# Chemical118/TREW

Hardware: NVIDIA B200
Metric: Gbases/s for trew short 5 32 at 1/2/4/8 B200; % of HBM roofline (higher is better)
Workload: dtype u64

## Files before the change

### trew_b200/csrc/device_ctx.cu

```cuda
#include <algorithm>
#include <chrono>
#include <cstdarg>
#include <cstdio>
#include <cstdlib>
#include <cstring>
#include <string>
#include <thread>
#include <vector>

#include <cuda_runtime.h>

#include "host_internal.h"
#include "scan_kernels.cuh"

using namespace trew;

namespace {

template <typename T, bool Pinned = false>
struct Buf {
    T* p = nullptr;
    size_t cap = 0;
    Buf() = default;
    Buf(Buf&& o) noexcept : p(o.p), cap(o.cap) { o.p = nullptr; o.cap = 0; }
    Buf(const Buf&) = delete;
    Buf& operator=(const Buf&) = delete;
    ~Buf() { release(); }
    cudaError_t grow(size_t n, cudaStream_t st) {
        if (n <= cap) return cudaSuccess;
        if (p) { cudaError_t e = cudaStreamSynchronize(st); if (e != cudaSuccess) return e; }
        return alloc(std::max((n + n / 4) * sizeof(T), (size_t)1 << 20) / sizeof(T));
    }
    cudaError_t alloc(size_t n) {
        cudaError_t e = release();
        if (e == cudaSuccess) e = Pinned ? cudaHostAlloc((void**)&p, n * sizeof(T), cudaHostAllocDefault) : cudaMalloc((void**)&p, n * sizeof(T));
        if (e != cudaSuccess) p = nullptr;
        else cap = n;
        return e;
    }
    cudaError_t release() {
        cudaError_t e = cudaSuccess;
        if (p) e = Pinned ? cudaFreeHost(p) : cudaFree(p);
        p = nullptr; cap = 0;
        return e;
    }
};

constexpr int kScanCounters = 8;
struct ScanBufs {
    Buf<unsigned int> survivors, counters;
    Buf<unsigned char> scratch;
    cudaError_t alloc(uint32_t n_units) {
        cudaError_t e = survivors.alloc(2 * (size_t)std::max<uint32_t>(n_units, 1));
        return e == cudaSuccess ? counters.alloc(kScanCounters) : e;
    }
};

struct SlotRes {
    Buf<unsigned char, true> h_buf;
    Buf<unsigned char> d_buf;
    Buf<unsigned char, true> h_inv;
    Buf<unsigned char> d_inv;
    size_t inv_cap = 0;
    Buf<unsigned int, true> h_keys;
    ScanBufs scan;
    size_t survivors_cap = 0;
    cudaStream_t stream = nullptr;
    cudaEvent_t ev_start = nullptr, ev_done = nullptr;
    bool in_flight = false;
};

struct RangeInfo { uint32_t r0, r1; uint64_t bases; uint32_t max_len; };

}

struct trew_resident {
    Buf<unsigned char> d_buf;
    DevBatch batch{};
    uint32_t n_reads = 0, n_units = 0, max_read_len = 0;
    uint64_t bases = 0;
    ScanBufs scan;
    cudaEvent_t ev[4] = {nullptr, nullptr, nullptr, nullptr};
    bool ev_pending = false;
};

struct trew_ctx {
    trew_config cfg{};
    int sm_count = 0;
    LaunchPlan plan{};
    cudaStream_t aux_stream = nullptr;
    cudaEvent_t ev_join = nullptr;
    int resident_streams = 1;
    uint64_t resident_seq = 0;
    DevCfg dcfg{};
    size_t n_slots = 0;
    Buf<Slot> table;
// ... 457 lines not shown
    return check_batch(nullptr, mode, batch);
}

static thread_local std::string g_create_error;

static int default_host_threads(int asked) {
    return asked > 0 ? asked : (int)std::min(64u, std::max(1u, std::thread::hardware_concurrency()));
}

const char* trew_dev_last_error(const trew_ctx* ctx) { return ctx ? ctx->err.c_str() : g_create_error.c_str(); }

static int create_ctx(const trew_config* cfg, trew_ctx** out, std::string& g_create_error, Pool* shared_pool) {
    if (!cfg || !out) return TREW_ERR_ARG;
    *out = nullptr;
    g_create_error.clear();
    auto bad_arg = [&](const char* msg) { g_create_error = msg; return TREW_ERR_ARG; };
    if (cfg->mode < 0 || cfg->mode > 2) return bad_arg("mode must be TREW_MODE_SHORT, _PAIR or _LONG");
    if (cfg->min_mer < 3 || cfg->max_mer > 64 || cfg->min_mer > cfg->max_mer) return bad_arg("need 3 <= MIN_MER <= MAX_MER <= 64");
    if (!(0 < cfg->low_baseline && cfg->low_baseline <= 1) || !(0 < cfg->high_baseline && cfg->high_baseline <= 1) ||
        cfg->low_baseline > cfg->high_baseline) return bad_arg("need 0 < LOW_BASELINE <= HIGH_BASELINE <= 1");
    if (cfg->mode == TREW_MODE_LONG && cfg->slice_length > 0 && cfg->slice_length < 2 * cfg->max_mer)
        return bad_arg("SLICE_LENGTH must be greater than or equal to twice of MAX_MER.");
    if (cfg->mode == TREW_MODE_LONG && cfg->slice_length > 512)
        return bad_arg("SLICE_LENGTH above 512 is not supported by the GPU path (a slice of up to 2*SLICE_LENGTH-1 bases must fit "
                       "a 1023-base window); use -s 512 or less.");
    trew_ctx* ctx = new trew_ctx();
    ctx->cfg = *cfg;
    if (ctx->cfg.slice_length <= 0) ctx->cfg.slice_length = 150;
    auto bail = [&](int rc) { g_create_error = ctx->err; trew_dev_destroy(ctx); return rc; };
#define CKC(call)                                                                                   \
    do {                                                                                            \
        cudaError_t e_ = (call);                                                                    \
        if (e_ != cudaSuccess) { fail(ctx, TREW_ERR_CUDA, "%s: %s", #call, cudaGetErrorString(e_)); return bail(TREW_ERR_CUDA); } \
    } while (0)
    const bool timing = getenv("TREW_CLI_TIMING") != nullptr;
    auto now = [] { return std::chrono::duration<double, std::milli>(std::chrono::steady_clock::now().time_since_epoch()).count(); };
    double t_prev = now();
    auto lap = [&](const char* what) {
        if (!timing) return;
        const double t = now();
        fprintf(stderr, "[trew] create, device %d: %s %.1f ms\n", cfg->device, what, t - t_prev);
        t_prev = t;
    };
    int ndev = 0;
    CKC(cudaGetDeviceCount(&ndev));
    lap("driver init");
    if (cfg->device < 0 || cfg->device >= ndev) { fail(ctx, TREW_ERR_CUDA, "no CUDA device %d (found %d)", cfg->device, ndev); return bail(TREW_ERR_CUDA); }
    CKC(cudaSetDevice(cfg->device));
    cudaDeviceProp prop;
    CKC(cudaGetDeviceProperties(&prop, cfg->device));
    ctx->sm_count = prop.multiProcessorCount;
    ctx->plan = default_launch_plan(ctx->sm_count);
    {
        auto env_int = [](const char* name, int dflt) { const char* e = getenv(name); return e && *e ? atoi(e) : dflt; };
        int v;
        if ((v = env_int("TREW_GRID_SCREEN", 0)) > 0) ctx->plan.screen_blocks = ctx->sm_count * v;
        if ((v = env_int("TREW_GRID_DECIDE", 0)) > 0) ctx->plan.decide_blocks = ctx->sm_count * v;
        if ((v = env_int("TREW_GRID_EXACT", 0)) > 0) ctx->plan.exact_blocks = std::min(ctx->plan.exact_blocks, ctx->sm_count * v);
        ctx->resident_streams = env_int("TREW_RESIDENT_STREAMS", 1) >= 2 ? 2 : 1;
        ctx->sparse_val = env_int("TREW_DENSE_VAL", 0) == 0;
        ctx->exact_flags = (unsigned int)env_int("TREW_EXACT_FLAGS", 0);
    }
    int lg = cfg->table_log2_slots > 0 ? cfg->table_log2_slots : 22;
    if (lg < 10 || lg > 28) { fail(ctx, TREW_ERR_ARG, "table_log2_slots out of range"); return bail(TREW_ERR_ARG); }
    ctx->n_slots = (size_t)1 << lg;
    CKC(ctx->table.alloc(ctx->n_slots));
    CKC(cudaMemset(ctx->table.p, 0, ctx->n_slots * sizeof(Slot)));
    lap("primary context + count table");
    CKC(ctx->d_error.alloc(2));
    CKC(cudaMemset(ctx->d_error.p, 0, 2 * sizeof(unsigned int)));
    CKC(ctx->d_total_surv.alloc(1));
    CKC(cudaMemset(ctx->d_total_surv.p, 0, sizeof(unsigned long long)));
    std::vector<unsigned short> thr;
    build_thr(cfg->low_baseline, thr);
    std::vector<unsigned short> thr_hi;
    build_thr(cfg->high_baseline, thr_hi);
    CKC(ctx->d_thr.alloc(2 * thr.size()));
    CKC(cudaMemcpy(ctx->d_thr.p, thr.data(), thr.size() * sizeof(unsigned short), cudaMemcpyHostToDevice));
    CKC(cudaMemcpy(ctx->d_thr.p + thr.size(), thr_hi.data(), thr_hi.size() * sizeof(unsigned short), cudaMemcpyHostToDevice));
    ctx->dcfg.mode = cfg->mode; ctx->dcfg.min_mer = cfg->min_mer; ctx->dcfg.max_mer = cfg->max_mer;
    ctx->dcfg.slice_len = ctx->cfg.slice_length; ctx->dcfg.low = cfg->low_baseline; ctx->dcfg.high = cfg->high_baseline;
    ctx->dcfg.slots = ctx->table.p; ctx->dcfg.slot_mask = (unsigned int)(ctx->n_slots - 1);
    ctx->dcfg.error_flag = ctx->d_error.p; ctx->dcfg.thr_low = ctx->d_thr.p; ctx->dcfg.thr_high = ctx->d_thr.p + kThrTableSize;
    CKC(prepare_exact(kMaxWindow + 9));
    lap("kernel attributes (module load)");
    CKC(cudaStreamCreateWithFlags(&ctx->main_stream, cudaStreamNonBlocking));
    CKC(cudaStreamCreateWithFlags(&ctx->aux_stream, cudaStreamNonBlocking));
    CKC(cudaEventCreateWithFlags(&ctx->ev_join, cudaEventDisableTiming));
    CKC(cudaEventCreate(&ctx->ev_a));
    CKC(cudaEventCreate(&ctx->ev_b));
    CKC(cudaEventCreate(&ctx->ev_t0));
    CKC(cudaEventCreate(&ctx->ev_t1));
    ctx->staging_bytes = cfg->staging_bytes ? (size_t)cfg->staging_bytes : ((size_t)64 << 20);
    int ns = cfg->n_staging > 0 ? cfg->n_staging : 3;
    ctx->slots.resize((size_t)ns);
    for (auto& s : ctx->slots) {
        CKC(s.h_buf.alloc(ctx->staging_bytes));
        CKC(s.d_buf.alloc(ctx->staging_bytes));
        s.inv_cap = ctx->staging_bytes / 8 / kInvRecBytes;
        CKC(s.h_inv.alloc((s.inv_cap + 1) * kInvRecBytes));
        CKC(s.d_inv.alloc((s.inv_cap + 1) * kInvRecBytes));
        CKC(s.h_keys.alloc(1));
        *s.h_keys.p = 0;
        s.survivors_cap = ctx->staging_bytes / 8;
        CKC(s.scan.alloc((uint32_t)s.survivors_cap));
        CKC(cudaStreamCreateWithFlags(&s.stream, cudaStreamNonBlocking));
        CKC(cudaEventCreate(&s.ev_start));
        CKC(cudaEventCreate(&s.ev_done));
    }
    CKC(ctx->d_n.alloc(1));
    lap("staging ring (pinned + device buffers)");
    if (shared_pool) { ctx->pool = shared_pool; ctx->own_pool = false; }
    else ctx->pool = new Pool(default_host_threads(cfg->host_threads));
#undef CKC
    *out = ctx;
    return TREW_OK;
}

int trew_dev_create(const trew_config* cfg, trew_ctx** out) { return create_ctx(cfg, out, g_create_error, nullptr); }

void trew_dev_destroy(trew_ctx* ctx) {
    if (!ctx) return;
    cudaSetDevice(ctx->cfg.device);
    cudaDeviceSynchronize();
    for (auto& s : ctx->slots) {
        if (s.stream) cudaStreamDestroy(s.stream);
        if (s.ev_start) cudaEventDestroy(s.ev_start);
        if (s.ev_done) cudaEventDestroy(s.ev_done);
    }
    if (ctx->main_stream) cudaStreamDestroy(ctx->main_stream);
    if (ctx->aux_stream) cudaStreamDestroy(ctx->aux_stream);
    if (ctx->ev_join) cudaEventDestroy(ctx->ev_join);
    if (ctx->ev_a) cudaEventDestroy(ctx->ev_a);
    if (ctx->ev_b) cudaEventDestroy(ctx->ev_b);
    if (ctx->ev_t0) cudaEventDestroy(ctx->ev_t0);
    if (ctx->ev_t1) cudaEventDestroy(ctx->ev_t1);
    if (ctx->own_pool) delete ctx->pool;
    delete ctx;
}

int trew_dev_submit_chunk(trew_ctx* ctx, const char* buffer1, const int32_t* locs1, uint32_t n1,
                          const char* buffer2, const int32_t* locs2, uint32_t n2) {
    if (!ctx) return TREW_ERR_ARG;
    CK(cudaSetDevice(ctx->cfg.device));
    const bool pair = ctx->cfg.mode == TREW_MODE_PAIR;
    if (pair ? (!buffer2 && n2) : (buffer2 != nullptr || n2 != 0)) return fail(ctx, TREW_ERR_ARG, "second chunk only in pair mode");
    if ((n1 && (!buffer1 || !locs1)) || (n2 && !locs2)) return fail(ctx, TREW_ERR_ARG, "null chunk");
    ChunkView cv{{buffer1, buffer2}, {locs1, locs2}, {nullptr, nullptr}, pair ? 2u : 1u};
    const uint32_t n = pair ? 2u * std::min(n1, n2) : n1;
    if (n == 0) return TREW_OK;
    for (int sd = 0; sd < (pair ? 2 : 1); sd++) {
        const int32_t* l = cv.locs[sd];
        uint32_t cnt = pair ? n / 2 : n;
        int32_t last = l[2 * (size_t)(cnt - 1) + 1];
        if (last >= l[2 * (size_t)(cnt - 1)]) cv.end[sd] = cv.buf[sd] + last + 1;
    }
    return submit_chunk_view(ctx, cv, n);
}

int trew_dev_submit_packed(trew_ctx* ctx, const trew_batch* batch) {
    if (!ctx || !batch) return TREW_ERR_ARG;
    int rc = check_batch(ctx, ctx->cfg.mode, batch);
    if (rc) return rc;
    CK(cudaSetDevice(ctx->cfg.device));
    uint32_t n = batch->n_reads;
    if (n == 0) return TREW_OK;
// ... 629 lines not shown
```

### trew_b200/csrc/scan_kernels.cu

```cuda
#include "scan_kernels.cuh"
#include "exact_thread.cuh"

#include <cstdio>

namespace trew {

typedef unsigned int u32;
typedef unsigned long long u64;
typedef unsigned __int128 u128;


__device__ __forceinline__ u32 lane_id() { return threadIdx.x & 31; }

__device__ __forceinline__ u32 low_mask(int bits) {
    return bits >= 32 ? 0xffffffffu : ((1u << bits) - 1u);
}

__device__ __forceinline__ u32 prefix_xor32(u32 x) {
    x ^= x << 1; x ^= x << 2; x ^= x << 4; x ^= x << 8; x ^= x << 16;
    return x;
}

__device__ __forceinline__ u64 mix64(u64 x) {
    x ^= x >> 33; x *= 0xff51afd7ed558ccdULL; x ^= x >> 33; x *= 0xc4ceb9fe1a85ec53ULL; x ^= x >> 33;
    return x;
}


__device__ __noinline__ void table_add_impl(Slot* slots, u32 slot_mask, u32* error_flag, u32 meta, u64 lo, u64 hi, u64 cnt) {
#ifdef TREW_EXP_NOADD
    return;
#endif
    u64 h = mix64(lo ^ mix64(hi + 0x9e3779b97f4a7c15ULL * (u64)(meta + 1)));
    u32 i = (u32)h & slot_mask;
    for (u32 probe = 0; probe <= slot_mask; probe++, i = (i + 1) & slot_mask) {
        Slot* s = slots + i;
        const uint4 a = __ldcg(reinterpret_cast<const uint4*>(s)), c = __ldcg(reinterpret_cast<const uint4*>(s) + 1);
        u32 st = c.w;
        if (st == 2u) {
            if (c.z == meta && a.x == (u32)lo && a.y == (u32)(lo >> 32) && a.z == (u32)hi && a.w == (u32)(hi >> 32)) {
                atomicAdd(&s->count, cnt);
                return;
            }
            __threadfence();
            if (__ldcg(&s->meta) == meta && __ldcg(&s->seq_lo) == lo && __ldcg(&s->seq_hi) == hi) {
                atomicAdd(&s->count, cnt);
                return;
            }
            continue;
        }
        int outcome = 0;
        do {
            st = atomicCAS(&s->state, 0u, 1u);
            if (st == 0u) {
                s->seq_lo = lo; s->seq_hi = hi; s->meta = meta;
                __threadfence();
                atomicExch(&s->state, 2u);
                atomicAdd(&s->count, cnt);
                atomicAdd(error_flag + 1, 1u);
                outcome = 1;
            } else if (st == 2u) {
                __threadfence();
                if (__ldcg(&s->meta) == meta && __ldcg(&s->seq_lo) == lo && __ldcg(&s->seq_hi) == hi) {
                    atomicAdd(&s->count, cnt);
                    outcome = 1;
                } else outcome = 2;
            }
        } while (outcome == 0);
        if (outcome == 1) return;
    }
    atomicExch(error_flag, 3u);
}

__device__ __forceinline__ void rec_append(UnitRecs* R, u64 unit, int table, int k, u64 lo, u64 hi, u64 count) {
    const u32 act = __activemask(), lane = threadIdx.x & 31;
    const int leader = __ffs(act) - 1;
    u64 base = 0;
    if ((int)lane == leader) base = atomicAdd(&R->n, (u64)__popc(act));
    base = __shfl_sync(act, base, leader);
    const u64 i = base + (u64)__popc(act & ((1u << lane) - 1u));
    if (i < R->cap) {
        uint4* p = reinterpret_cast<uint4*>(R->buf + i);
        p[0] = make_uint4((u32)unit, (u32)(unit >> 32), (u32)lo, (u32)(lo >> 32));
        p[1] = make_uint4((u32)hi, (u32)(hi >> 32), (u32)count, (u32)table | ((u32)k << 8));
// ... 202 lines not shown
        csa(x[0], x[1], x[2], s1, c1); csa(x[3], x[4], x[5], s2, c2); csa(s1, s2, x[6], s3, c3);
        csa(c1, c2, c3, s4, c4);
        return __popc(s3) + __popc(x[7]) + 2 * __popc(s4) + 4 * __popc(c4);
    } else {
        int t = 0;
#pragma unroll
        for (int j = 0; j < NW; j++) t += __popc(x[j]);
        return t;
    }
}

template <int NW>
__device__ __noinline__ bool probe_filter(const DevBatch& b, u32 pos, int wl, int k0, int k1,
                                          const unsigned short* __restrict__ thr) {
    u32 PH[NW], PL[NW], QH[NW], QL[NW], WV[NW];
    {
        u32 t[NW];
        load_bits<NW>(b.hi, pos, t); prefix_xor_excl<NW>(t, PH);
        load_bits<NW>(b.lo, pos, t); prefix_xor_excl<NW>(t, PL);
        load_bits<NW>(b.val, pos, WV); mask_bits<NW>(WV, wl);
    }
    shr_var<NW>(PH, k0, QH);
    shr_var<NW>(PL, k0, QL);
    sliding_and<NW>(WV, k0);
    u32 PA[NW];
    bool have_pa = false;
    for (int k = k0; k <= k1; k++) {
        u32 a[NW], bb[NW], c[NW];
#pragma unroll
        for (int j = 0; j < NW; j++) {
            u32 dh = QH[j] ^ PH[j], dl = QL[j] ^ PL[j];
            a[j] = dh & WV[j]; bb[j] = dl & WV[j]; c[j] = a[j] & dl;
        }
        int T = popc_multi<NW>(WV);
        if (T == 0) break;
        int cH = popc_multi<NW>(a), cL = popc_multi<NW>(bb), c11 = popc_multi<NW>(c);
        int c10 = cH - c11, c01 = cL - c11, c00 = T - cH - cL + c11;
        int U = max(max(c00, c01), max(c10, c11));
        int need = thr[T];
        if (U >= need) {
            u32 QA[NW];
            if (!have_pa) {
                u32 A[NW], t[NW];
                load_bits<NW>(b.hi, pos, A); load_bits<NW>(b.lo, pos, t);
#pragma unroll
                for (int j = 0; j < NW; j++) A[j] &= t[j];
                prefix_xor_excl<NW>(A, PA);
                have_pa = true;
            }
            shr_var<NW>(PA, k, QA);
            u32 x11[NW], x10[NW], x01[NW], x00[NW];
#pragma unroll
            for (int j = 0; j < NW; j++) {
                u32 da = QA[j] ^ PA[j];
                u32 dh = QH[j] ^ PH[j], dl = QL[j] ^ PL[j];
                x11[j] = c[j] & da; x10[j] = a[j] & ~dl & da; x01[j] = bb[j] & ~dh & da; x00[j] = WV[j] & ~dh & ~dl & da;
            }
            int n11 = popc_multi<NW>(x11), n10 = popc_multi<NW>(x10), n01 = popc_multi<NW>(x01), n00 = popc_multi<NW>(x00);
            int U2 = max(max(max(n11, c11 - n11), max(n10, c10 - n10)), max(max(n01, c01 - n01), max(n00, c00 - n00)));
            if (U2 >= need) return true;
        }
        shr1<NW>(QH); shr1<NW>(QL);
        u32 t[NW];
#pragma unroll
        for (int j = 0; j < NW; j++) t[j] = WV[j];
        shr1<NW>(t);
#pragma unroll
        for (int j = 0; j < NW; j++) WV[j] &= t[j];
    }
    return false;
}

template <int MAXNW>
__device__ __forceinline__ bool probe_dispatch(const DevBatch& b, const Probe& p, const unsigned short* thr) {
    if (p.k1 < p.k0) return false;
    int need_bits = p.wl + 1;
    if (need_bits <= 96) return probe_filter<3>(b, p.pos, p.wl, p.k0, p.k1, thr);
    if constexpr (MAXNW >= 5) { if (need_bits <= 160) return probe_filter<5>(b, p.pos, p.wl, p.k0, p.k1, thr); }
    if constexpr (MAXNW >= 8) { if (need_bits <= 256) return probe_filter<8>(b, p.pos, p.wl, p.k0, p.k1, thr); }
    return true;
}


constexpr u32 kPackC11 = 1u - (1u << 8) - (1u << 16) + (1u << 24);
constexpr u32 kPackH = (1u << 8) - (1u << 24);
constexpr u32 kPackL = (1u << 16) - (1u << 24);
#ifndef TREW_SCREEN_UNROLL
#define TREW_SCREEN_UNROLL 2
#endif
constexpr int kScreenUnroll = TREW_SCREEN_UNROLL;
constexpr int kFastMaxWl = 95;
constexpr int kFastTabSize = kFastMaxWl + 2;
constexpr int kProbeShift = 28;
constexpr int kMod4BelowWindows = 48;
constexpr int kThreadMinWindows = 36;

__device__ __forceinline__ uint4 fast_entry(int T, int need) {
    uint4 e = make_uint4(0u, 0u, 0u, 0u);
    if (T <= 0) return e;
    int T01 = min(T, 64);
    e.y = T >= 32 ? 0xffffffffu : ((1u << T) - 1u);
    e.z = T <= 32 ? 0u : (T >= 64 ? 0xffffffffu : ((1u << (T - 32)) - 1u));
    int np = need - (T - T01);
    if (np <= 0) e.x = 0x80808080u;
    else if (np > 64) e.x = (u32)T01 << 24;
    else e.x = ((u32)T01 << 24) + (u32)(128 - np) * 0x01010101u;
    return e;
}

template <int S>
__device__ __forceinline__ bool fast_span(const u32 (&ph)[5], const u32 (&pl)[5], int wl, int ka, int kb,
                                          const uint4* __restrict__ tab) {
    const uint4* tp = tab + (wl - ka + 1);
#pragma unroll (kScreenUnroll)
    for (int k = ka; k <= kb; k++, tp--) {
        const uint4 e = *tp;
        u32 qh0 = __funnelshift_r(ph[S], ph[S + 1], k), qh1 = __funnelshift_r(ph[S + 1], ph[S + 2], k);
        u32 ql0 = __funnelshift_r(pl[S], pl[S + 1], k), ql1 = __funnelshift_r(pl[S + 1], pl[S + 2], k);
        u32 a0 = (qh0 ^ ph[0]) & e.y, a1 = (qh1 ^ ph[1]) & e.z;
        u32 b0 = (ql0 ^ pl[0]) & e.y, b1 = (ql1 ^ pl[1]) & e.z;
        u32 x = e.x + (u32)(__popc(a0) + __popc(a1)) * kPackH + (u32)(__popc(b0) + __popc(b1)) * kPackL +
                (u32)(__popc(a0 & b0) + __popc(a1 & b1)) * kPackC11;
        if (x & 0x80808080u) return true;
    }
    return false;
}

__device__ __forceinline__ bool probe_is_fast(const Probe& p) { return p.wl <= kFastMaxWl && p.k1 <= 63 && p.k1 <= p.wl; }

__device__ __forceinline__ bool screen_probe(const DevBatch& b, const Probe& p, const uint4* __restrict__ tab) {
    if (p.k1 < p.k0) return false;
    if (!probe_is_fast(p)) return true;
    u32 t[3], full[3] = {0xffffffffu, 0xffffffffu, 0xffffffffu};
    mask_bits<3>(full, p.wl);
    load_bits<3>(b.val, p.pos, t);
    if ((((t[0] & full[0]) ^ full[0]) | ((t[1] & full[1]) ^ full[1]) | ((t[2] & full[2]) ^ full[2])) != 0u) return true;
    u32 ph[5], pl[5], q[3];
    load_bits<3>(b.hi, p.pos, t); mask_bits<3>(t, p.wl); prefix_xor_excl<3>(t, q);
    ph[0] = q[0]; ph[1] = q[1]; ph[2] = q[2]; ph[3] = 0u; ph[4] = 0u;
    load_bits<3>(b.lo, p.pos, t); mask_bits<3>(t, p.wl); prefix_xor_excl<3>(t, q);
    pl[0] = q[0]; pl[1] = q[1]; pl[2] = q[2]; pl[3] = 0u; pl[4] = 0u;
    int k0 = p.k0;
    if (k0 < 32) {
        if (fast_span<0>(ph, pl, p.wl, k0, min(p.k1, 31), tab)) return true;
        k0 = 32;
    }
    return p.k1 >= 32 && fast_span<1>(ph, pl, p.wl, k0, p.k1, tab);
}

constexpr int kFastMaxWlLong = 159;
constexpr int kFastTabSizeLong = kFastMaxWlLong + 2;
struct __align__(16) FastEntryLong { u32 base, m0, m1, m2, m3, pad0, pad1, pad2; };

__device__ __forceinline__ FastEntryLong fast_entry_long(int T, int need) {
    FastEntryLong e = {0u, 0u, 0u, 0u, 0u, 0u, 0u, 0u};
    if (T <= 0) return e;
    const int T01 = min(T, 128);
    u32 m[4];
#pragma unroll
    for (int j = 0; j < 4; j++) { int vb = T - 32 * j; m[j] = vb <= 0 ? 0u : low_mask(min(32, vb)); }
    e.m0 = m[0]; e.m1 = m[1]; e.m2 = m[2]; e.m3 = m[3];
    const int np = need - (T - T01);
    if (np <= 0) e.base = 0x80808080u;
    else if (np > 128) e.base = 0u;
    else e.base = ((u32)T01 << 24) + (u32)(128 - np) * 0x01010101u;
    return e;
}

template <int S>
__device__ __forceinline__ bool fast_span_long(const u32 (&ph)[8], const u32 (&pl)[8], int wl, int ka, int kb,
                                               const FastEntryLong* __restrict__ tab) {
    const FastEntryLong* tp = tab + (wl - ka + 1);
    for (int k = ka; k <= kb; k++, tp--) {
        const uint4 e0 = *reinterpret_cast<const uint4*>(tp);
        const u32 m3 = tp->m3;
        if (e0.x == 0u) continue;
        const u32 mk[4] = {e0.y, e0.z, e0.w, m3};
        int cH = 0, cL = 0, c11 = 0;
#pragma unroll
        for (int j = 0; j < 4; j++) {
            u32 a = (__funnelshift_r(ph[S + j], ph[S + j + 1], k) ^ ph[j]) & mk[j];
            u32 bb = (__funnelshift_r(pl[S + j], pl[S + j + 1], k) ^ pl[j]) & mk[j];
            cH += __popc(a); cL += __popc(bb); c11 += __popc(a & bb);
        }
        u32 x = e0.x + (u32)cH * kPackH + (u32)cL * kPackL + (u32)c11 * kPackC11;
        if (x & 0x80808080u) return true;
    }
    return false;
}

__device__ __forceinline__ bool probe_is_fast_long(const Probe& p) { return p.wl <= kFastMaxWlLong && p.k1 <= 64 && p.k1 <= p.wl; }

__device__ __noinline__ bool screen_probe_long(const DevBatch& b, const Probe& p, const FastEntryLong* __restrict__ tab) {
    u32 t[5], full[5] = {0xffffffffu, 0xffffffffu, 0xffffffffu, 0xffffffffu, 0xffffffffu};
    mask_bits<5>(full, p.wl);
    load_bits<5>(b.val, p.pos, t);
    u32 bad = 0;
#pragma unroll
    for (int j = 0; j < 5; j++) bad |= (t[j] & full[j]) ^ full[j];
    if (bad) return true;
    u32 ph[8], pl[8], q[5];
    load_bits<5>(b.hi, p.pos, t); mask_bits<5>(t, p.wl); prefix_xor_excl<5>(t, q);
#pragma unroll
    for (int j = 0; j < 8; j++) ph[j] = j < 5 ? q[j] : 0u;
    load_bits<5>(b.lo, p.pos, t); mask_bits<5>(t, p.wl); prefix_xor_excl<5>(t, q);
#pragma unroll
    for (int j = 0; j < 8; j++) pl[j] = j < 5 ? q[j] : 0u;
    int k0 = p.k0;
    if (k0 < 32) {
        if (fast_span_long<0>(ph, pl, p.wl, k0, min(p.k1, 31), tab)) return true;
        k0 = 32;
    }
    if (k0 < 64 && p.k1 >= 32) {
        if (fast_span_long<1>(ph, pl, p.wl, k0, min(p.k1, 63), tab)) return true;
        k0 = 64;
    }
    return p.k1 >= 64 && fast_span_long<2>(ph, pl, p.wl, k0, p.k1, tab);
}

__device__ __forceinline__ void list_append(bool flag, u32 value, u32* __restrict__ list, u32* __restrict__ count) {
    u32 m = __ballot_sync(0xffffffffu, flag);
    if (m) {
        u32 base = 0;
        if (lane_id() == 0) base = atomicAdd(count, (u32)__popc(m));
        base = __shfl_sync(0xffffffffu, base, 0);
        if (flag) list[base + __popc(m & ((1u << lane_id()) - 1u))] = value;
    }
}

__device__ __forceinline__ void list_append_rev(bool flag, u32 value, u32* __restrict__ top, u32* __restrict__ count) {
    u32 m = __ballot_sync(0xffffffffu, flag);
    if (m) {
        u32 base = 0;
        if (lane_id() == 0) base = atomicAdd(count, (u32)__popc(m));
        base = __shfl_sync(0xffffffffu, base, 0);
        if (flag) *(top - (base + __popc(m & ((1u << lane_id()) - 1u)))) = value;
    }
}

#ifndef TREW_SCREEN_BPS
#define TREW_SCREEN_BPS 8
#endif
template <bool LONG>
__global__ void __launch_bounds__(256, LONG ? 4 : TREW_SCREEN_BPS) trew_screen_kernel(DevCfg cfg, DevBatch b, u32 n_units,
                                                                                     u32* __restrict__ deferred, u32* __restrict__ n_deferred) {
    __shared__ uint4 tab[kFastTabSize];
    __shared__ FastEntryLong tab_long[LONG ? kFastTabSizeLong : 1];
    for (int T = threadIdx.x; T < kFastTabSize; T += blockDim.x) tab[T] = fast_entry(T, (int)cfg.thr_low[T]);
    if (LONG) for (int T = threadIdx.x; T < kFastTabSizeLong; T += blockDim.x) tab_long[T] = fast_entry_long(T, (int)cfg.thr_low[T]);
    __syncthreads();
    u32 stride = gridDim.x * blockDim.x;
    u32 n_round = (n_units + 31u) & ~31u;
    for (u32 u = blockIdx.x * blockDim.x + threadIdx.x; u < n_round; u += stride) {
        u32 pm = 0;
        if (u < n_units) {
            Probe p[4];
            int np = unit_probes(cfg, b, u, p);
            for (int i = 0; i < np; i++) {
                bool d;
                if (LONG && p[i].k1 >= p[i].k0 && !probe_is_fast(p[i]) && probe_is_fast_long(p[i])) d = screen_probe_long(b, p[i], tab_long);
                else d = screen_probe(b, p[i], tab);
                pm |= d ? 1u << i : 0u;
            }
        }
        list_append(pm != 0, u | (pm << kProbeShift), deferred, n_deferred);
    }
}

__device__ __forceinline__ int max4(int a, int b, int c, int d) { return max(max(a, b), max(c, d)); }

__device__ __forceinline__ u32 shr3(const u32 (&p)[3], int j, int k) {
    const int s = k >> 5;
    const u32 lo = j + s < 3 ? (s ? (j == 0 ? p[1] : p[2]) : p[j]) : 0u;
    const u32 hi = j + s + 1 < 3 ? (s ? p[2] : (j == 0 ? p[1] : p[2])) : 0u;
    return __funnelshift_r(lo, hi, k);
}
constexpr int kDecideThreads = 256;
__device__ __noinline__ bool mod4_level(const DevBatch& b, u32 pos, int wl, int k, int need, u32 pass8, u32 wv0, u32 wv1, u32 wv2, u32* cache,
                                        bool& cached) {
    const u32 wv[3] = {wv0, wv1, wv2};
    u32 p0[3][3], p1[3][3];
    if (!cached) {
        u32 x[3][3];
        load_bits<3>(b.hi, pos, x[0]); mask_bits<3>(x[0], wl);
        load_bits<3>(b.lo, pos, x[1]); mask_bits<3>(x[1], wl);
#pragma unroll
        for (int j = 0; j < 3; j++) x[2][j] = x[0][j] & x[1][j];
#pragma unroll
        for (int p = 0; p < 3; p++) {
            prefix_xor_excl<3>(x[p], p0[p]);
            u32 c[3];
#pragma unroll
            for (int j = 0; j < 3; j++) c[j] = x[p][j] & p0[p][j];
            prefix_xor_excl<3>(c, p1[p]);
#pragma unroll
            for (int j = 0; j < 3; j++) { cache[(6 * p + j) * kDecideThreads] = p0[p][j]; cache[(6 * p + 3 + j) * kDecideThreads] = p1[p][j]; }
        }
        cached = true;
    } else {
#pragma unroll
        for (int p = 0; p < 3; p++)
#pragma unroll
            for (int j = 0; j < 3; j++) { p0[p][j] = cache[(6 * p + j) * kDecideThreads]; p1[p][j] = cache[(6 * p + 3 + j) * kDecideThreads]; }
    }
    u32 d0[3][3], d1[3][3];
#pragma unroll
    for (int p = 0; p < 3; p++) {
#pragma unroll
        for (int j = 0; j < 3; j++) {
            const u32 q0 = shr3(p0[p], j, k);
            d0[p][j] = q0 ^ p0[p][j];
            d1[p][j] = shr3(p1[p], j, k) ^ p1[p][j] ^ (~q0 & p0[p][j]);
        }
    }
#pragma unroll 1
    for (int c2 = 0; c2 < 8; c2++) {
        if (!((pass8 >> c2) & 1u)) continue;
        u32 mw[3];
        int cnt = 0;
#pragma unroll
        for (int j = 0; j < 3; j++) {
            mw[j] = wv[j] & (d0[0][j] ^ ((c2 & 1) ? 0u : ~0u)) & (d0[1][j] ^ ((c2 & 2) ? 0u : ~0u)) & (d0[2][j] ^ ((c2 & 4) ? 0u : ~0u));
            cnt += __popc(mw[j]);
        }
        if (cnt < need) continue;
        bool may = true;
#pragma unroll
        for (int p = 0; p < 3 && may; p++) {
            const int one = __popc(mw[0] & d1[p][0]) + __popc(mw[1] & d1[p][1]) + __popc(mw[2] & d1[p][2]);
            const int zero = cnt - one;
            if (min(one, zero) >= need) return true;
            const u32 flip = one >= zero ? 0u : ~0u;
#pragma unroll
            for (int j = 0; j < 3; j++) mw[j] &= d1[p][j] ^ flip;
            cnt = max(one, zero);
            may = cnt >= need;
        }
        if (may) return true;
    }
    return false;
}

template <int S>
__device__ __forceinline__ bool decide_span(const u32 (&ph)[5], const u32 (&pl)[5], const u32 (&pa)[5], u32 (&wv)[3], int ka, int kb,
// ... 1334 lines not shown
```

### trew_b200/csrc/scan_kernels.cuh

```cuda
#pragma once
#include <cstdint>
#include <cuda_runtime.h>

#include "../../include/trew_b200.h"

namespace trew {

constexpr int kThrTableSize = 1025;
constexpr int kMaxWindow = 1023;

struct __align__(32) Slot {
    unsigned long long seq_lo;
    unsigned long long seq_hi;
    unsigned long long count;
    unsigned int meta;
    unsigned int state;
};

struct UnitRecs {
    trew_unit_record* buf;
    unsigned long long cap;
    unsigned long long n;
};

struct DevCfg {
    int mode, min_mer, max_mer, slice_len;
    double low, high;
    Slot* slots;
    unsigned int slot_mask;
    unsigned int* error_flag;
    const unsigned short* thr_low;
    const unsigned short* thr_high;
    UnitRecs* recs;
    unsigned long long unit_base;
};

struct DevBatch {
    unsigned int n_reads;
    const unsigned int* bit_off;
    const unsigned int* hi;
    const unsigned int* lo;
    const unsigned int* val;
};

struct ExactArgs {
    const unsigned int* survivors;
    const unsigned int* n_survivors;
    unsigned int* work_counter;
    unsigned char* slice_scratch;
    unsigned int slice_scratch_stride;
    int run_cap;
    unsigned long long* total_survivors;
    int packed_probes;
    int reverse;
    unsigned int exp_flags;
};

struct LaunchPlan { int screen_blocks, decide_blocks, exact_blocks; };
LaunchPlan default_launch_plan(int sm_count);

void launch_filter(const DevCfg& cfg, const DevBatch& b, unsigned int n_units, unsigned int max_read_len,
                   unsigned int* deferred, unsigned int* n_deferred, unsigned int* survivors, unsigned int* n_survivors,
                   const LaunchPlan& plan, cudaStream_t stream, cudaEvent_t after_screen,
                   unsigned int* surv_b_top, unsigned int* n_surv_b, unsigned int* work_counter);
size_t exact_smem_bytes(int run_cap, bool wide);
cudaError_t prepare_exact(int run_cap_max);
void launch_exact(const DevCfg& cfg, const DevBatch& b, const ExactArgs& a, const LaunchPlan& plan, cudaStream_t stream);
int exact_warps_total(int sm_count);
bool long_thread_path_applies(const DevCfg& cfg);
size_t long_thread_scratch_bytes(unsigned int s_cap, unsigned int max_slices);
void launch_long_thread(const DevCfg& cfg, const DevBatch& b, const unsigned int* survivors, const unsigned int* n_survivors,
                        int packed_probes, unsigned int s_cap, unsigned int max_slices, unsigned char* scratch, unsigned int* hard,
                        unsigned int* n_hard, unsigned long long* total_survivors, int sm_count, cudaStream_t stream);
bool thread_path_applies(const DevCfg& cfg, unsigned int max_read_len);
void launch_exact_thread(const DevCfg& cfg, const DevBatch& b, const unsigned int* survivors, const unsigned int* n_survivors,
                         int packed_probes, unsigned int* hard, unsigned int* n_hard, unsigned long long* total_survivors, int sm_count,
                         int blocks_per_sm, unsigned int* work_counter, cudaStream_t stream);
void launch_compact(const Slot* slots, unsigned int n_slots, trew_entry* out, unsigned int* d_n, cudaStream_t stream, unsigned int cap);
cudaError_t sort_entries_radix(const trew_entry* d_entries, trew_entry* d_out, unsigned int n, bool wide, void* d_temp,
                               size_t* temp_bytes, cudaStream_t stream);
cudaError_t combine_sorted_rows(const trew_entry* d_sorted, unsigned int n, trew_entry* d_out, unsigned int* d_n_out, void* d_temp,
                                size_t* temp_bytes, cudaStream_t stream);
cudaError_t filter_report_rows(const trew_entry* d_rows, unsigned int n, unsigned int min_total, trew_entry* d_out, unsigned int* d_n_out,
                               void* d_temp, size_t* temp_bytes, cudaStream_t stream);
void launch_clear_invalid(unsigned int* val, const unsigned int* rec, unsigned int n, cudaStream_t stream);
void launch_merge_entries(const DevCfg& cfg, const trew_entry* entries, unsigned int n, cudaStream_t stream);

cudaError_t sort_combine_records(const trew_unit_record* d_in, unsigned int n, bool wide, trew_unit_record* d_out, unsigned int* d_n_out,
                                 void* d_temp, size_t* temp_bytes, cudaStream_t stream);

void launch_synth(unsigned long long seed, unsigned int n_reads, unsigned int read_len, unsigned int tel_thr,
                  unsigned int half_thr, unsigned int n_thr, unsigned int sub_thr, unsigned int flavor, unsigned int* bit_off,
                  unsigned int* hi, unsigned int* lo, unsigned int* val, size_t plane_words, cudaStream_t stream);

}
```

Measured before the change: 1035.

## Add majority-side bound screening path for small periods in fast screen

Adds a cheaper per-period test for periods where the required match count exceeds half the period. It counts only the majority side and one masked popcount, dropping one popcount pair and a multiply. The host picks the period range, or odd periods only, where this applies. The span loop is specialised per template with a manual two-way unroll, which adds code size and branch complexity to the screen kernel.

Result: faster. 1065 (median of 6 runs) (+2.8%).

```diff
diff --git a/trew_b200/csrc/device_ctx.cu b/trew_b200/csrc/device_ctx.cu
--- a/trew_b200/csrc/device_ctx.cu
+++ b/trew_b200/csrc/device_ctx.cu
@@ -12,6 +12,7 @@
 
 #include "host_internal.h"
 #include "scan_kernels.cuh"
+#include "screen_bound.cuh"
 
 using namespace trew;
 
@@ -635,6 +636,11 @@
     ctx->dcfg.slice_len = ctx->cfg.slice_length; ctx->dcfg.low = cfg->low_baseline; ctx->dcfg.high = cfg->high_baseline;
     ctx->dcfg.slots = ctx->table.p; ctx->dcfg.slot_mask = (unsigned int)(ctx->n_slots - 1);
     ctx->dcfg.error_flag = ctx->d_error.p; ctx->dcfg.thr_low = ctx->d_thr.p; ctx->dcfg.thr_high = ctx->d_thr.p + kThrTableSize;
+    {
+        bool odd = false;
+        sb::major_split<2>(thr.data(), sb::kFastMaxT, &ctx->dcfg.screen_major_t, &odd);
+        ctx->dcfg.screen_major_odd = odd ? 1 : 0;
+    }
     CKC(prepare_exact(kMaxWindow + 9));
     lap("kernel attributes (module load)");
     CKC(cudaStreamCreateWithFlags(&ctx->main_stream, cudaStreamNonBlocking));
diff --git a/trew_b200/csrc/scan_kernels.cu b/trew_b200/csrc/scan_kernels.cu
--- a/trew_b200/csrc/scan_kernels.cu
+++ b/trew_b200/csrc/scan_kernels.cu
@@ -1,5 +1,6 @@
 #include "scan_kernels.cuh"
 #include "exact_thread.cuh"
+#include "screen_bound.cuh"
 
 #include <cstdio>
 
@@ -368,53 +369,50 @@
 }
 
 
-constexpr u32 kPackC11 = 1u - (1u << 8) - (1u << 16) + (1u << 24);
-constexpr u32 kPackH = (1u << 8) - (1u << 24);
-constexpr u32 kPackL = (1u << 16) - (1u << 24);
-#ifndef TREW_SCREEN_UNROLL
-#define TREW_SCREEN_UNROLL 2
-#endif
-constexpr int kScreenUnroll = TREW_SCREEN_UNROLL;
 constexpr int kFastMaxWl = 95;
 constexpr int kFastTabSize = kFastMaxWl + 2;
+static_assert(kFastTabSize - 1 == sb::kFastMaxT, "the host picks the majority-side periods over the table's T range");
 constexpr int kProbeShift = 28;
 constexpr int kMod4BelowWindows = 48;
 constexpr int kThreadMinWindows = 36;
 
-__device__ __forceinline__ uint4 fast_entry(int T, int need) {
-    uint4 e = make_uint4(0u, 0u, 0u, 0u);
-    if (T <= 0) return e;
-    int T01 = min(T, 64);
-    e.y = T >= 32 ? 0xffffffffu : ((1u << T) - 1u);
-    e.z = T <= 32 ? 0u : (T >= 64 ? 0xffffffffu : ((1u << (T - 32)) - 1u));
-    int np = need - (T - T01);
-    if (np <= 0) e.x = 0x80808080u;
-    else if (np > 64) e.x = (u32)T01 << 24;
-    else e.x = ((u32)T01 << 24) + (u32)(128 - np) * 0x01010101u;
-    return e;
-}
-
-template <int S>
+__device__ __forceinline__ uint4 fast_entry(int T, int need, bool major) {
+    u32 m[2], base, t01;
+    sb::make_entry<2>(T, need, major, base, m, t01);
+    return make_uint4(base, m[0], m[1], t01);
+}
+
+template <int S, bool MAJOR>
+__device__ __forceinline__ bool fast_period(const u32 (&ph)[5], const u32 (&pl)[5], int k, const uint4 e) {
+    const u32 a[2] = {(__funnelshift_r(ph[S], ph[S + 1], k) ^ ph[0]) & e.y, (__funnelshift_r(ph[S + 1], ph[S + 2], k) ^ ph[1]) & e.z};
+    const u32 b[2] = {(__funnelshift_r(pl[S], pl[S + 1], k) ^ pl[0]) & e.y, (__funnelshift_r(pl[S + 1], pl[S + 2], k) ^ pl[1]) & e.z};
+    return MAJOR ? sb::major_pass<2>(e.x, e.w, a, b) : sb::bucket_pass<2>(e.x, a, b);
+}
+
+template <int S, bool F0, bool F1>
 __device__ __forceinline__ bool fast_span(const u32 (&ph)[5], const u32 (&pl)[5], int wl, int ka, int kb,
                                           const uint4* __restrict__ tab) {
     const uint4* tp = tab + (wl - ka + 1);
-#pragma unroll (kScreenUnroll)
-    for (int k = ka; k <= kb; k++, tp--) {
-        const uint4 e = *tp;
-        u32 qh0 = __funnelshift_r(ph[S], ph[S + 1], k), qh1 = __funnelshift_r(ph[S + 1], ph[S + 2], k);
-        u32 ql0 = __funnelshift_r(pl[S], pl[S + 1], k), ql1 = __funnelshift_r(pl[S + 1], pl[S + 2], k);
-        u32 a0 = (qh0 ^ ph[0]) & e.y, a1 = (qh1 ^ ph[1]) & e.z;
-        u32 b0 = (ql0 ^ pl[0]) & e.y, b1 = (ql1 ^ pl[1]) & e.z;
-        u32 x = e.x + (u32)(__popc(a0) + __popc(a1)) * kPackH + (u32)(__popc(b0) + __popc(b1)) * kPackL +
-                (u32)(__popc(a0 & b0) + __popc(a1 & b1)) * kPackC11;
-        if (x & 0x80808080u) return true;
-    }
-    return false;
+    int k = ka;
+    for (; k < kb; k += 2, tp -= 2) {
+        if (fast_period<S, F0>(ph, pl, k, tp[0])) return true;
+        if (fast_period<S, F1>(ph, pl, k + 1, tp[-1])) return true;
+    }
+    return k == kb && fast_period<S, F0>(ph, pl, k, tp[0]);
+}
+
+template <int S>
+__device__ __forceinline__ bool fast_range(const u32 (&ph)[5], const u32 (&pl)[5], int wl, int ka, int kb, int ks, bool odd_only,
+                                           const uint4* __restrict__ tab) {
+    if (fast_span<S, false, false>(ph, pl, wl, ka, min(kb, ks - 1), tab)) return true;
+    ka = max(ka, ks);
+    if (!odd_only) return fast_span<S, true, true>(ph, pl, wl, ka, kb, tab);
+    return ((wl - ka + 1) & 1) ? fast_span<S, true, false>(ph, pl, wl, ka, kb, tab) : fast_span<S, false, true>(ph, pl, wl, ka, kb, tab);
 }
 
 __device__ __forceinline__ bool probe_is_fast(const Probe& p) { return p.wl <= kFastMaxWl && p.k1 <= 63 && p.k1 <= p.wl; }
 
-__device__ __forceinline__ bool screen_probe(const DevBatch& b, const Probe& p, const uint4* __restrict__ tab) {
+__device__ __forceinline__ bool screen_probe(const DevBatch& b, const Probe& p, const uint4* __restrict__ tab, int major_t, bool odd_only) {
     if (p.k1 < p.k0) return false;
     if (!probe_is_fast(p)) return true;
     u32 t[3], full[3] = {0xffffffffu, 0xffffffffu, 0xffffffffu};
@@ -426,12 +424,13 @@
     ph[0] = q[0]; ph[1] = q[1]; ph[2] = q[2]; ph[3] = 0u; ph[4] = 0u;
     load_bits<3>(b.lo, p.pos, t); mask_bits<3>(t, p.wl); prefix_xor_excl<3>(t, q);
     pl[0] = q[0]; pl[1] = q[1]; pl[2] = q[2]; pl[3] = 0u; pl[4] = 0u;
+    const int ks = p.wl - major_t + 1;
     int k0 = p.k0;
     if (k0 < 32) {
-        if (fast_span<0>(ph, pl, p.wl, k0, min(p.k1, 31), tab)) return true;
+        if (fast_range<0>(ph, pl, p.wl, k0, min(p.k1, 31), ks, odd_only, tab)) return true;
         k0 = 32;
     }
-    return p.k1 >= 32 && fast_span<1>(ph, pl, p.wl, k0, p.k1, tab);
+    return p.k1 >= 32 && fast_range<1>(ph, pl, p.wl, k0, p.k1, ks, odd_only, tab);
 }
 
 constexpr int kFastMaxWlLong = 159;
@@ -469,7 +468,7 @@
             u32 bb = (__funnelshift_r(pl[S + j], pl[S + j + 1], k) ^ pl[j]) & mk[j];
             cH += __popc(a); cL += __popc(bb); c11 += __popc(a & bb);
         }
-        u32 x = e0.x + (u32)cH * kPackH + (u32)cL * kPackL + (u32)c11 * kPackC11;
+        u32 x = e0.x + (u32)cH * sb::kPackH + (u32)cL * sb::kPackL + (u32)c11 * sb::kPackC11;
         if (x & 0x80808080u) return true;
     }
     return false;
@@ -532,7 +531,8 @@
                                                                                      u32* __restrict__ deferred, u32* __restrict__ n_deferred) {
     __shared__ uint4 tab[kFastTabSize];
     __shared__ FastEntryLong tab_long[LONG ? kFastTabSizeLong : 1];
-    for (int T = threadIdx.x; T < kFastTabSize; T += blockDim.x) tab[T] = fast_entry(T, (int)cfg.thr_low[T]);
+    for (int T = threadIdx.x; T < kFastTabSize; T += blockDim.x)
+        tab[T] = fast_entry(T, (int)cfg.thr_low[T], sb::major_at(T, cfg.screen_major_t, cfg.screen_major_odd != 0));
     if (LONG) for (int T = threadIdx.x; T < kFastTabSizeLong; T += blockDim.x) tab_long[T] = fast_entry_long(T, (int)cfg.thr_low[T]);
     __syncthreads();
     u32 stride = gridDim.x * blockDim.x;
@@ -545,7 +545,7 @@
             for (int i = 0; i < np; i++) {
                 bool d;
                 if (LONG && p[i].k1 >= p[i].k0 && !probe_is_fast(p[i]) && probe_is_fast_long(p[i])) d = screen_probe_long(b, p[i], tab_long);
-                else d = screen_probe(b, p[i], tab);
+                else d = screen_probe(b, p[i], tab, cfg.screen_major_t, cfg.screen_major_odd != 0);
                 pm |= d ? 1u << i : 0u;
             }
         }
diff --git a/trew_b200/csrc/scan_kernels.cuh b/trew_b200/csrc/scan_kernels.cuh
--- a/trew_b200/csrc/scan_kernels.cuh
+++ b/trew_b200/csrc/scan_kernels.cuh
@@ -31,6 +31,8 @@
     unsigned int* error_flag;
     const unsigned short* thr_low;
     const unsigned short* thr_high;
+    int screen_major_t;
+    int screen_major_odd;
     UnitRecs* recs;
     unsigned long long unit_base;
 };
diff --git a/trew_b200/csrc/screen_bound.cuh b/trew_b200/csrc/screen_bound.cuh
--- /dev/null
+++ b/trew_b200/csrc/screen_bound.cuh
@@ -0,0 +1,94 @@
+#pragma once
+#include <stdint.h>
+
+#if defined(__CUDACC__)
+#define SB_HD __host__ __device__ __forceinline__
+#else
+#define SB_HD inline
+#endif
+
+namespace trew {
+namespace sb {
+
+typedef uint32_t u32;
+
+SB_HD int popc(u32 x) {
+#if defined(__CUDA_ARCH__)
+    return __popc(x);
+#else
+    return __builtin_popcount(x);
+#endif
+}
+SB_HD u32 fshr(u32 lo, u32 hi, int sh) {
+#if defined(__CUDA_ARCH__)
+    return __funnelshift_r(lo, hi, sh);
+#else
+    sh &= 31;
+    return sh ? (lo >> sh) | (hi << (32 - sh)) : lo;
+#endif
+}
+
+constexpr u32 kPackC11 = 1u - (1u << 8) - (1u << 16) + (1u << 24);
+constexpr u32 kPackH = (1u << 8) - (1u << 24);
+constexpr u32 kPackL = (1u << 16) - (1u << 24);
+constexpr u32 kPackSide = 1u << 8;
+constexpr u32 kPackB1 = 1u - (1u << 8);
+
+constexpr int kFastMaxT = 96;
+
+SB_HD bool major_applies(int T01, int np) { return 2 * np > T01; }
+
+template <int NW>
+SB_HD void make_entry(int T, int need, bool major, u32& base, u32 (&m)[NW], u32& t01) {
+    base = 0u; t01 = 0u;
+    for (int j = 0; j < NW; j++) {
+        const int vb = T - 32 * j;
+        m[j] = vb <= 0 ? 0u : (vb >= 32 ? 0xffffffffu : (1u << vb) - 1u);
+    }
+    if (T <= 0) return;
+    const int T01 = T < 32 * NW ? T : 32 * NW, np = need - (T - T01);
+    t01 = (u32)T01;
+    if (major) {
+        base = (u32)(128 - np) * 0x0101u;
+    } else if (np <= 0) {
+        base = 0x80808080u;
+    } else if (np > 32 * NW) {
+        base = NW > 2 ? 0u : (u32)T01 << 24;
+    } else {
+        base = ((u32)T01 << 24) + (u32)(128 - np) * 0x01010101u;
+    }
+}
+
+template <int NW>
+SB_HD bool bucket_pass(u32 base, const u32 (&a)[NW], const u32 (&b)[NW]) {
+    int cH = 0, cL = 0, c11 = 0;
+    for (int j = 0; j < NW; j++) { cH += popc(a[j]); cL += popc(b[j]); c11 += popc(a[j] & b[j]); }
+    return ((base + (u32)cH * kPackH + (u32)cL * kPackL + (u32)c11 * kPackC11) & 0x80808080u) != 0u;
+}
+
+template <int NW>
+SB_HD bool major_pass(u32 base, u32 t01, const u32 (&a)[NW], const u32 (&b)[NW]) {
+    int cH = 0;
+    for (int j = 0; j < NW; j++) cH += popc(a[j]);
+    const bool a0_side = 2u * (u32)cH < t01;
+    const u32 flip = a0_side ? 0xffffffffu : 0u;
+    const int side = a0_side ? (int)t01 - cH : cH;
+    int nb1 = 0;
+    for (int j = 0; j < NW; j++) nb1 += popc(b[j] & (a[j] ^ flip));
+    return ((base + (u32)side * kPackSide + (u32)nb1 * kPackB1) & 0x8080u) != 0u;
+}
+
+template <int NW>
+inline void major_split(const unsigned short* thr, int tcap, int* tmax, bool* odd_only) {
+    auto applies = [&](int T) { const int T01 = T < 32 * NW ? T : 32 * NW; return major_applies(T01, (int)thr[T] - (T - T01)); };
+    int all = 0, odd = 0;
+    while (all < tcap && applies(all + 1)) all++;
+    while (odd < tcap && ((odd + 1) % 2 == 0 || applies(odd + 1))) odd++;
+    if (all >= (odd + 1) / 2) { *tmax = all; *odd_only = false; }
+    else { *tmax = odd; *odd_only = true; }
+}
+
+SB_HD bool major_at(int T, int tmax, bool odd_only) { return T >= 1 && T <= tmax && (!odd_only || (T & 1)); }
+
+}
+}
```
